# timothijoe/LightZero

Measured on AMD Instinct MI355X. Metric: MCTS simulations/sec (whole node), 256 parallel envs x 50 sims/step, higher is better.
Workload: dtype f32; 1 GPU; CartPole-v0 MuZero search, MuZeroModelMLP (latent 128, support 601), 256 envs x 50 sims per GPU; global_batch=256, num_simulations=50, rng=glibc, step=graph, hip_graph=True, heads=random, parallelism=env-sharded x1

## Files before the change

lightzero_amd/csrc/lzm_search_res.h:

```cpp
#pragma once
#include <hip/hip_runtime.h>
#include <stdint.h>

#include "lzm_search_mlp.h"
#include "lzm_tree.h"

namespace lzm {

constexpr int kRT = 256;
constexpr int kRWaves = kRT / 64;
constexpr int kRHid = 128, kRF = 32, kRV = 601;
constexpr int kRMaxA = 32;
constexpr int kRTail = kRV - 2 * kRT;
static_assert(kRTail > 0 && 2 * kRTail <= kRT, "support tail: two lanes per column");
constexpr int kRSlotsD = 16, kRSlotsRH = 4, kRSlotsVPH = 8, kRSlotsS = 20, kRSlotsPO = 1;

constexpr int kDwinBack = 20;

__device__ __forceinline__ void dwin_add_part(const uint32_t *coef, int npos, const uint32_t *z0, int lo, uint32_t *win,
                                              int part) {
  const int lane = threadIdx.x & 63;
  const int q = lo + lane;
  const int j0 = 11 * part, j1 = part == 2 ? 31 : j0 + 11;
  if (q < npos) {
// ... 628 lines not shown
    const int d = (lane == 0 && tv > 0) ? tv : tv + 1;
    const float y = div_small_y(d), nd = -(float)d;
    const bool below = lane < pend;
    float qv = parent_q;
    for (int i = pend; i < upto; ++i) {
      const float in = __int_as_float(__builtin_amdgcn_update_dpp(0, __float_as_int(qv), 0x138, 0xF, 0xF, true));
      const float q = div_small_core(in + tq, y, nd);
      qv = below ? qv : q;
    }
    const unsigned long long range = (~0ull >> (64 - (upto - pend))) << pend;
    const unsigned long long bad = __builtin_amdgcn_ballot_w64(__builtin_amdgcn_classf(tq, 0x020) ||
                                                               __builtin_amdgcn_classf(qv, sgpr_literal<0x207>()));
    if ((bad & range) == 0ull) return readlane_f(qv, upto - 1);
    parent_q = pend > 0 ? readlane_f(qv, pend - 1) : 0.0f;
  }
  const auto level = [&](int l, float &tq) {
    const int Ls = __builtin_amdgcn_readlane(plev, l);
    tq = readlane_f(rtq, Ls);
    return (__builtin_amdgcn_readlane(rpk, Ls) >> 5) & 3;
  };
  int l = pend;
  if (l == 0) {
    float tq;
    const int tv = level(0, tq);
    parent_q = div_small(tv > 0 ? tq : parent_q + tq, tv > 0 ? tv : 1);
    l = 1;
  }
  for (; l < upto; ++l) {
    float tq;
    const int tv = level(l, tq);
    parent_q = div_small(parent_q + tq, tv + 1);
  }
  return parent_q;
}

template <bool CLASSIFY, typename Draw>
__device__ inline Descent descend_a2r(const TreeView &t, const A2Rec &rc, bool leaf_ok, float4 mm, int vtp, int players,
                                      const int *rleg, int nleg, Draw draw, TieInfo *tie, WalkState *at_tie = nullptr) {
  const int lane = threadIdx.x & 63;
  const int dmax = t.depth_cap - 1;
  const int lat0 = __builtin_amdgcn_readfirstlane(t.meta[0].latent);
  int lat = lat0, len = 0;
  int plev = 0, pact = 0;
  float parent_q = 0.0f;
  int pend = 0;
  const auto rl = [](int v, int l) { return __builtin_amdgcn_readlane(v, l); };
  const auto rlf = [](float v, int l) { return __int_as_float(__builtin_amdgcn_readlane(__float_as_int(v), l)); };
  const auto child = [](int pk, int j) { return (int)((unsigned)pk << (8 - 8 * j)) >> 24; };
  const auto decided = [](int pk) { return (int)((unsigned)pk << 16) >> 24; };
  auto step = [&](int action, int nlat) {
    plev = lane == len ? lat : plev;
    pact = lane == len ? action : pact;
    ++len;
    lat = nlat;
  };
  const auto plat_of = [&]() { return len > 0 ? rl(plev, len - 1) : -1; };
  const auto act_of = [&]() { return len > 0 ? rl(pact, len - 1) : -1; };
  auto settle = [&](int upto) {
    parent_q = settle_chain(rc.tq, rc.pk, plev, leaf_ok, pend, upto, parent_q);
    pend = upto > pend ? upto : pend;
  };
  auto flush = [&]() {
    if (lane == 0) t.path[0] = 0;
    if (lane < len) {
      t.path_act[lane] = pact;
      t.path[lane + 1] = 1 + 2 * plev + pact;
    }
  };
  if (CLASSIFY) tie->status = 0;
  int pk = 0, dl = 0;
  bool stop = false;
  if (lat >= 0 && len < dmax) {
    pk = rl(rc.pk, lat);
    dl = pk & 7;
    if (dl <= 1)
      step(rleg[dl], decided(pk));
    else
      stop = true;
  }
  for (;;) {
    if (!stop && lat >= 0) {
      for (;;) {
        pk = rl(rc.pk, lat);
        dl = pk & 7;
        if (dl > 1) {
          stop = true;
          break;
        }
        step(dl, decided(pk));
        if (lat < 0) break;
      }
    }
    if (!stop || len >= dmax) break;
    stop = false;
    const bool root = len == 0;
    int jsel = 0;
    if (dl == 4 && leaf_ok) {
      if (CLASSIFY) {
        flush();
        const int vt = (players > 1 && (len & 1)) ? ((vtp == 1) ? 2 : 1) : vtp;
        tie->status = 1;
        tie->level = len;
        tie->mask = 3ull;
        Descent d;
        d.len = len + 1;
        d.x = lat;
        d.action = -1;
        d.vtp = players > 1 ? ((vt == 1) ? 2 : 1) : vt;
        d.leaf = -1;
        return d;
      }
      jsel = __builtin_amdgcn_readfirstlane((int)(draw(len) % 2u));
    } else {
      settle(len);
      bool tie2 = dl == 3;
      float mean_q = 0.0f;
      if (dl != 3) {
        const float delta = mm.x - mm.y;
        const bool scale = delta > 0;
        const float div = (delta < mm.z) ? mm.z : delta;
        const float tq = rlf(rc.tq, lat);
        const int tv = (pk >> 5) & 3;
        const bool rootq = root && tv > 0;
        mean_q = div_small(rootq ? tq : parent_q + tq, rootq ? tv : tv + 1);
        float vu = mm_norm_fixed(scale, mm.y, div, mean_q);
        if (vu < 0) vu = 0;
        if (vu > 1) vu = 1;
        const float s0 = rlf(rc.x0, lat) + ((pk & 8) ? rlf(rc.y0, lat) : vu);
        const float s1 = rlf(rc.x1, lat) + ((pk & 16) ? rlf(rc.y1, lat) : vu);
        const float M = fmaxf(s0, s1);
        const int j = (s0 == M) ? 0 : 1;
        jsel = __builtin_amdgcn_readfirstlane(j);
        tie2 = __builtin_amdgcn_readfirstlane((j == 0 && s1 >= M - 0.000001f) ? 1 : 0) != 0;
      }
      if (CLASSIFY && tie2) {
        const int vt = (players > 1 && (len & 1)) ? ((vtp == 1) ? 2 : 1) : vtp;
        const bool all_leaves = ((unsigned)pk >> 16) == 0xffffu;
        if (at_tie && !all_leaves) {
          const int plat = plat_of(), last_action = act_of();
          at_tie->node = root ? 0 : 1 + 2 * plat + last_action; at_tie->lat = lat; at_tie->len = len; at_tie->plat = plat;
          at_tie->last_action = last_action; at_tie->is_root = root; at_tie->vtp = vt; at_tie->parent_q = parent_q;
        }
        flush();
        tie->status = all_leaves ? 1 : 2;
        tie->level = len;
        tie->mask = 3ull;
        Descent d;
        d.len = len + 1;
        d.x = lat;
        d.action = -1;
        d.vtp = players > 1 ? ((vt == 1) ? 2 : 1) : vt;
        d.leaf = -1;
        return d;
      }
      if (!CLASSIFY && tie2) jsel = __builtin_amdgcn_readfirstlane((int)(draw(len) % 2u));
      if (dl != 3) {
        parent_q = mean_q;
        pend = len + 1;
      }
    }
    step(root ? rleg[jsel] : jsel, child(pk, jsel));
  }
  flush();
  const int plat = plat_of(), last_action = act_of();
  Descent d;
  d.len = len;
  d.x = plat;
  d.action = last_action;
  d.vtp = (players > 1 && (len & 1)) ? ((vtp == 1) ? 2 : 1) : vtp;
  d.leaf = len == 0 ? 0 : 1 + 2 * plat + last_action;
  return d;
}

struct NoSide {
  __device__ __forceinline__ void operator()(int) const {}
};
template <int NR, typename WF, typename SF = NoSide>
__device__ __forceinline__ void dense128n(const float *x, WF w, float *z, SF side = SF()) {
  const int e = threadIdx.x & 7;
  float4 xv[NR][4];
#pragma unroll
  for (int r = 0; r < NR; ++r)
#pragma unroll
    for (int j = 0; j < 4; ++j) xv[r][j] = reinterpret_cast<const float4 *>(x + r * kRRow)[4 * e + (e >> 2) + j];
  float a[NR][4][4];
#pragma unroll
  for (int r = 0; r < NR; ++r)
#pragma unroll
    for (int c = 0; c < 4; ++c) a[r][c][0] = a[r][c][1] = a[r][c][2] = a[r][c][3] = 0.0f;
#pragma unroll
  for (int j = 0; j < 4; ++j)
#pragma unroll
    for (int c = 0; c < 4; ++c) {
      side(4 * j + c);
      const float4 q = w(4 * j + c);
#pragma unroll
      for (int r = 0; r < NR; ++r) fma4(xv[r][j], q, a[r][c]);
    }
#pragma unroll
  for (int r = 0; r < NR; ++r)
    z[r] = reduce_d4((a[r][0][0] + a[r][0][1]) + (a[r][0][2] + a[r][0][3]),
                     (a[r][1][0] + a[r][1][1]) + (a[r][1][2] + a[r][1][3]),
                     (a[r][2][0] + a[r][2][1]) + (a[r][2][2] + a[r][2][3]),
                     (a[r][3][0] + a[r][3][1]) + (a[r][3][2] + a[r][3][3]));
}

template <int NH>
__device__ __forceinline__ void support_decode_n(const float (*z)[3], float *red, float *out) {
  const int tid = threadIdx.x, lane = tid & 63, wid = tid >> 6;
  const bool ok2 = tid < 2 * kRTail && !(tid & 1);
#pragma unroll
  for (int h = 0; h < NH; ++h) {
    float m = fmaxf(z[h][0], z[h][1]);
    if (ok2) m = fmaxf(m, z[h][2]);
    m = wave_max_dpp(m);
    if (lane == 0) red[4 * h + wid] = m;
  }
  __syncthreads();
  const float half = (float)((kRV - 1) / 2);
  const float j0 = (float)tid - half, j1 = (float)(kRT + tid) - half, j2 = (float)(2 * kRT + (tid >> 1)) - half;
#pragma unroll
  for (int h = 0; h < NH; ++h) {
    const float M = fmaxf(fmaxf(red[4 * h], red[4 * h + 1]), fmaxf(red[4 * h + 2], red[4 * h + 3]));
    const float e0 = expf(z[h][0] - M), e1 = expf(z[h][1] - M), e2 = ok2 ? expf(z[h][2] - M) : 0.0f;
    float se = (e0 + e1) + e2, sj = (e0 * j0 + e1 * j1) + e2 * j2;
    se = wave_sum(se);
    sj = wave_sum(sj);
    if (lane == 0) {
      red[4 * NH + 8 * h + wid] = se;
      red[4 * NH + 8 * h + 4 + wid] = sj;
    }
  }
  __syncthreads();
#pragma unroll
  for (int h = 0; h < NH; ++h) {
    const float *q = red + 4 * NH + 8 * h;
    out[h] = h_inverse(((q[4] + q[5]) + (q[6] + q[7])) / ((q[0] + q[1]) + (q[2] + q[3])));
  }
}

__device__ inline void resolve_tie(const TreeView &t, int A, int lvl, unsigned long long m, uint32_t rr, int *act) {
  int kk = (int)(rr % (uint32_t)__popcll(m));
  for (; kk > 0; --kk) m &= m - 1;
  const int jsel = __ffsll((long long)m) - 1;
  const int parent = t.path[lvl];
  const int action = legal_at(t, 0, parent, jsel);
  t.path_act[lvl] = action;
  t.path[lvl + 1] = 1 + A * t.meta[parent].latent + action;
  *act = action;
}

__device__ inline int lookback_sum(const SearchArgs &p, int k, int g, int G, unsigned long long epoch, int *part) {
  const int lane = threadIdx.x & 63;
  int sum = 0;
  for (int q = threadIdx.x; q < g; q += kRT) {
    unsigned long long v;
    long long spins = 0;
    while (true) {
      v = __hip_atomic_load(&p.flags[(size_t)k * G + q], __ATOMIC_RELAXED, __HIP_MEMORY_SCOPE_AGENT);
      if ((v >> 32) == epoch) break;
      if (++spins > (1ll << 22)) {
        atomicAdd(p.diag, 1);
        v = 0;
        break;
      }
      __builtin_amdgcn_s_sleep(1);
    }
    sum += (int)(v & 0xffffffffu);
  }
  sum = xor_sum(sum);
  if (lane == 0) part[threadIdx.x >> 6] = sum;
  __syncthreads();
  return (part[0] + part[1]) + (part[2] + part[3]);
}

__device__ inline int lookback_sum_w0(const SearchArgs &p, int k, int g, int G, unsigned long long epoch) {
  const int lane = threadIdx.x & 63;
  const unsigned long long ok = epoch << 32;
  unsigned long long v[4];
#pragma unroll
  for (int j = 0; j < 4; ++j) {
    const int q = lane + 64 * j;
    v[j] = q < g ? __hip_atomic_load(&p.flags[(size_t)k * G + q], __ATOMIC_RELAXED, __HIP_MEMORY_SCOPE_AGENT) : ok;
  }
  float sum = 0.0f;
#pragma unroll
  for (int j = 0; j < 4; ++j) {
    const int q = lane + 64 * j;
    long long spins = 0;
    while ((v[j] >> 32) != epoch) {
      if (++spins > (1ll << 22)) {
        atomicAdd(p.diag, 1);
        v[j] = ok;
        break;
      }
      __builtin_amdgcn_s_sleep(1);
      v[j] = __hip_atomic_load(&p.flags[(size_t)k * G + q], __ATOMIC_RELAXED, __HIP_MEMORY_SCOPE_AGENT);
    }
    sum += (float)(int)(v[j] & 0xffffffffu);
  }
  return (int)wave_sum(sum);
}

constexpr int kResStaticBytes = (kRRow + 4 * kRRow + 2 * (4 * kRRow + kRF + 2 * kRF + kRMaxA) + kResBiasFloats) * 4 + 2048;
constexpr int kResMaxBytes = 160 * 1024 - kResStaticBytes;
__host__ __device__ constexpr int res_round4(int x) { return (x + 3) & ~3; }
__host__ __device__ constexpr ResPlan res_plan(int cap, int lut_n, int depth_cap, int S, int A) {
  ResPlan q{};
  int o = 0;
  q.wd1 = o; o += kRSlotsD * kRT * 4;
  q.wd2 = o; o += kRSlotsD * kRT * 4;
  q.stat = o; o += cap * 4;
  q.meta = o; o += cap * 4;
  q.lut = o; o += res_round4(2 * lut_n);
  q.legal = o; o += res_round4(A + 1);
  q.val = o; o += res_round4(cap);
  q.path = o; o += res_round4(depth_cap);
  q.pact = o; o += res_round4(depth_cap);
  q.act = o; o += A * kRHid;
  q.l2n = o; o += res_round4(S + 2);
  q.nq = o; o += res_round4(2 * (S + 2));
  q.cs = o; o += 4 * cap;
  q.dec = o; o += res_round4(S + 2);
  q.misc = o; o += res_round4(S + 32);
  const int tri = res_round4(lut_n * (lut_n + 1) / 2);
  q.pbt = o;
  q.pbt_rows = ((o + tri) * 4 <= kResMaxBytes && tri <= 8192) ? lut_n : 0;
  if (q.pbt_rows) o += tri;
  q.floats = o;
  return q;
}

template <int SMODE, int RNG, bool STAMPS>
__global__ __launch_bounds__(kRT) __attribute__((amdgpu_waves_per_eu(1, 1))) void search_res_kernel(SearchArgs p, ResNet n) {
  if (!STAMPS) p.phase = nullptr;
  if (RNG >= 0) p.fast = RNG;
  const ResPlan L = n.plan;
  static_assert(SMODE == 1 || SMODE == 4 || SMODE == 5, "selection modes: 1, 4, 5");
  if ((SMODE == 4 || SMODE == 5) && RNG == 0 && !STAMPS) n.spec_depth = 1;
  extern __shared__ float4 smem4[];
  float *smem = reinterpret_cast<float *>(smem4);
  const int tid = threadIdx.x, g = blockIdx.x, G = gridDim.x, lane = tid & 63, wid = tid >> 6;
  const int B = p.B, A = p.A;
  const int i = g;
  unsigned long long stamp_ = p.phase ? __builtin_amdgcn_s_memtime() : 0ull;
  unsigned long long isub_ = stamp_;
#define LZM_ISTAMP(n)                                                      \
  do {                                                                     \
    if (p.phase && tid == 0) {                                             \
      const unsigned long long now_ = __builtin_amdgcn_s_memtime();       \
      s_phase[n] += (now_ - isub_) * (unsigned long long)p.S;              \
      isub_ = now_;                                                        \
    }                                                                      \
  } while (0)

  __shared__ uint32_t s_z0[31];
  __shared__ int s_players, s_epoch, s_x, s_act, s_status, s_tlevel, s_vtp;
  __shared__ int s_len[1], s_part[kRWaves], s_nlat;
  __shared__ unsigned long long s_tmask;
  __shared__ WalkState s_walk;
  __shared__ float4 s_mm;
  __shared__ float s_red[12 * 2];
  __shared__ uint32_t s_dwin[64];
  __shared__ int s_dlo, s_base_prev;
  if (tid == 0) { s_dlo = -1000000; s_base_prev = 0; }
  __shared__ uint64_t s_exptab[32];
  if (threadIdx.x < 32) s_exptab[threadIdx.x] = kExp2fTab[threadIdx.x];
  __shared__ unsigned long long s_phase[64];
  if (p.phase && tid < 64) s_phase[tid] = 0ull;
  unsigned long long s_wait = 0ull;

  TreeView t;
  t.A = A; t.cap = p.cap; t.lut_n = p.lut_n; t.depth_cap = p.depth_cap; t.B = 1;
  t.path = reinterpret_cast<int32_t *>(smem + L.path);
  t.path_act = reinterpret_cast<int32_t *>(smem + L.pact);
  t.pathlen = s_len;
  {
    NodeStat *ls = reinterpret_cast<NodeStat *>(smem + L.stat);
    NodeMeta *lm = reinterpret_cast<NodeMeta *>(smem + L.meta);
    float2 *llut = reinterpret_cast<float2 *>(smem + L.lut);
    int32_t *llegal = reinterpret_cast<int32_t *>(smem + L.legal);
    float *lval = smem + L.val;
    for (int e = tid; e < p.cap; e += kRT) {
      const NodeStat s = p.stat[(size_t)e * B + i];
      ls[e] = s;
      lm[e] = p.meta[(size_t)e * B + i];
      lval[e] = node_value(s);
    }
    for (int e = tid; e < p.lut_n; e += kRT) llut[e] = p.lut[e];
    float *lpbt = smem + L.pbt;
    build_pbt(p.lut, p.pbt_rows, lpbt, tid, kRT);
    for (int e = tid; e < A; e += kRT) llegal[e] = p.legal[(size_t)i * A + e];
    if (tid == 0) llegal[A] = p.nlegal[i];
    t.stat = ls; t.meta = lm; t.lut = llut; t.legal = llegal; t.nlegal = llegal + A; t.val = lval;
    t.pbt = p.pbt_rows ? lpbt : nullptr;
  }
  LZM_ISTAMP(24);
  int *L2N = reinterpret_cast<int *>(smem + L.l2n);
  float2 *NQ = reinterpret_cast<float2 *>(smem + L.nq);
  int *DEC = reinterpret_cast<int *>(smem + L.dec);
  float4 *CS = reinterpret_cast<float4 *>(smem + L.cs);
  for (int e = tid; e < p.S + 2; e += kRT) L2N[e] = e == 0 ? 0 : -1;
  if (tid == 0) s_nlat = 1;
  if (tid == 0) {
    s_mm = p.mm_fresh ? make_float4(kFloatMin, kFloatMax, p.mm_delta, 0.0f) : p.minmax[i];
    s_vtp = p.vtp_in[i];
    s_epoch = (int)__hip_atomic_load(p.epoch, __ATOMIC_RELAXED, __HIP_MEMORY_SCOPE_AGENT);
  }
  if (wid == 0) {
    int m = INT_MIN;
    for (int q = lane; q < B; q += 64) m = max(m, p.vtp_in[q]);
    m = xor_max(m);
    if (lane == 0) s_players = (m == -1) ? 1 : 2;
  }
  uint32_t *s_seeds = reinterpret_cast<uint32_t *>(smem + L.misc);
  uint32_t *s_pow = s_seeds + p.S;
  if (p.step_count) {
    const long long c = *p.step_count;
    for (int e = tid; e < p.S; e += kRT) s_seeds[e] = (uint32_t)((p.step_base + c * (long long)p.S + e) % 1000000ll);
  } else {
    for (int e = tid; e < p.S; e += kRT) s_seeds[e] = p.seeds[e];
  }
  if (!p.fast)
    for (int e = tid; e < 31; e += kRT) s_pow[e] = p.pow16807[e];

  LZM_ISTAMP(25);
  __shared__ float4 s_acts[(kRRow + 4 * kRRow + 4 * kRRow + kRF + 2 * kRF + kRMaxA) / 4];
  __shared__ float4 s_bias[kResBiasFloats / 4];
  float *X0 = reinterpret_cast<float *>(s_acts), *T1 = X0 + kRRow, *NL = T1 + 2 * kRRow, *T2 = NL + 2 * kRRow,
        *T3 = T2 + kRRow, *U2 = T3 + kRRow, *U3 = U2 + kRRow, *RHo = U3 + kRRow, *HV = RHo + kRF, *LG = HV + 2 * kRF;
  float *ACT = smem + L.act;
  const float4 *WD1 = reinterpret_cast<const float4 *>(smem + L.wd1);
  const float4 *WD2 = reinterpret_cast<const float4 *>(smem + L.wd2);
  {
    float4 st[kRSlotsD];
    res_fetch<kRSlotsD>(res_blk4(n, kRbD + 1), st);
#pragma unroll
    for (int j = 0; j < kRSlotsD; ++j) reinterpret_cast<float4 *>(smem + L.wd1)[j * kRT + tid] = st[j];
    res_fetch<kRSlotsD>(res_blk4(n, kRbD + 2), st);
#pragma unroll
    for (int j = 0; j < kRSlotsD; ++j) reinterpret_cast<float4 *>(smem + L.wd2)[j * kRT + tid] = st[j];
  }
  for (int e = tid; e < A * kRHid; e += kRT) ACT[e] = res_blk(n, kRbAct, A)[e];
  LZM_ISTAMP(26);
  float4 wD3[kRSlotsD], wD4[kRSlotsD], wRS[kRSlotsS], wRH[kRSlotsRH], wVPH[kRSlotsVPH], wPO[1];
  res_fetch<kRSlotsD>(res_blk4(n, kRbD + 3), wD3);
  res_fetch<kRSlotsD>(res_blk4(n, kRbD + 4), wD4);
  res_fetch<kRSlotsS>(res_blk4(n, kRbRS), wRS);
  res_fetch<kRSlotsRH>(res_blk4(n, kRbRH), wRH);
  res_fetch<kRSlotsVPH>(res_blk4(n, kRbVPH), wVPH);
  res_fetch<kRSlotsPO>(res_blk4(n, kRbPO), wPO);
  const int cD = d_col(), pD = tid & 1, cRH = tid >> 3, pRH = tid & 7, cVP = tid >> 2, pVP = tid & 3, cPO = tid >> 3;
  LZM_ISTAMP(27);
  float *BB = reinterpret_cast<float *>(s_bias);
  {
    constexpr int kNB = (kResBiasFloats + kRT - 1) / kRT;
    float bv[kNB];
    const float *bsrc = res_blk(n, kRbBD, A);
#pragma unroll
    for (int j = 0; j < kNB; ++j) bv[j] = j * kRT + tid < kResBiasFloats ? bsrc[j * kRT + tid] : 0.0f;
#pragma unroll
    for (int j = 0; j < kNB; ++j)
      if (j * kRT + tid < kResBiasFloats) BB[j * kRT + tid] = bv[j];
  }
  const float *BD = BB, *BRH = BD + 6 * kRHid, *BVP = BRH + kRF, *BRS = BVP + 2 * kRF,
              *BVS = BRS + ((kRV + 3) & ~3), *BPO = BVS + ((kRV + 3) & ~3);
  float4 P[kRSlotsS];
  res_fetch<kRSlotsD>(res_blk4(n, kRbD), P);
#pragma unroll
  for (int j = kRSlotsD; j < kRSlotsS; ++j) P[j] = make_float4(0.0f, 0.0f, 0.0f, 0.0f);
  __syncthreads();
  const int players = s_players;
  const unsigned long long epoch = (unsigned long long)(uint32_t)s_epoch;
  int rleg[2];
  const int nleg = t.nlegal[0];
#pragma unroll
  for (int j = 0; j < 2; ++j) rleg[j] = j < A ? t.legal[j] : 0;
  LZM_ISTAMP(28);
  LZM_STAMP(10);

  for (int k = 0; k < p.S; ++k) {
    const uint32_t seed = s_seeds[k];
    const bool regwalk = SMODE == 5;
    const int smode = regwalk ? 4 : (SMODE == 4 && A != 2) ? 1 : SMODE;
    A2Rec rc = {0, 0.0f, 0.0f, 0.0f, 0.0f, 0.0f};
    __syncthreads();
    if (regwalk) {
      if (tid < s_nlat + k) node_terms_a2(t, tid, L2N, NQ, CS, s_mm, players, p.disc, DEC, rleg, nleg, &rc);
    } else {
      if (smode == 4)
        precompute_terms_a2(t, s_nlat + k, L2N, NQ, CS, s_mm, players, p.disc, DEC, rleg, nleg);
      else
        precompute_terms(t, s_nlat + k, L2N, NQ, CS, s_mm, players, p.disc);
      __syncthreads();
    }
    LZM_STAMP(12);
    if (wid != 0 && k > 0) res_fetch<kRSlotsD>(res_blk4(n, kRbD), P);
    if (!p.fast && wid == 1) {
      const uint32_t sd = seed == 0 ? 1u : seed;
      if (sd < 0x7fffffffu) {
        if (lane < 31) {
          unsigned long long x = (unsigned long long)sd * s_pow[lane];
          unsigned long long r = (x & 0x7fffffffull) + (x >> 31);
          r = (r & 0x7fffffffull) + (r >> 31);
          if (r >= 0x7fffffffull) r -= 0x7fffffffull;
          s_z0[lane] = (uint32_t)r;
        }
      } else if (lane == 0) {
        glibc_seed_state(seed, s_z0);
      }
    }
    if (RNG != 1 && wid == 1) s_dwin[lane] = 0u;
    if (wid == 0) {
      const float4 mm = s_mm;
      int w_status = 0, w_x = 0;
      if (p.fast) {
        auto draw = [seed, i](int level) -> uint32_t {
          uint4 o = philox4x32_10(make_uint4((uint32_t)level, (uint32_t)i, 0u, 0u), make_uint2(seed, 0x4c5a4d43u));
          return o.x >> 1;
        };
        Descent d;
        if (regwalk) {
          d = descend_a2r<false>(t, rc, terms_finite_a2r(rc, mm), mm, s_vtp, players, rleg, nleg, draw, nullptr);
          w_x = d.x;
        } else if (smode == 4) {
          d = descend_a2f<false>(t, NQ, DEC, CS, mm, s_vtp, players, rleg, nleg, draw, nullptr);
        } else if (smode == 1) {
          d = descend_terms<false>(t, NQ, CS, mm, s_vtp, players, draw, nullptr);
        }
        if (lane == 0) { s_len[0] = d.len; s_x = d.x; s_act = d.action; s_status = 0; }
      } else {
        TieInfo ti;
        auto nodraw = [](int) -> uint32_t { return 0u; };
        Descent d;
        if (regwalk) {
          WalkState ws;
          d = descend_a2r<true>(t, rc, terms_finite_a2r(rc, mm), mm, s_vtp, players, rleg, nleg, nodraw, &ti, &ws);
          LZM_STAMP(13);
          if (lane == 0 && ti.status == 2) s_walk = ws;
          w_status = ti.status;
          w_x = d.x;
        } else if (smode == 4) {
          WalkState ws;
          d = descend_a2f<true>(t, NQ, DEC, CS, mm, s_vtp, players, rleg, nleg, nodraw, &ti, &ws);
          LZM_STAMP(13);
          if (lane == 0 && ti.status == 2) s_walk = ws;
        } else if (smode == 1) {
          WalkState ws;
          d = descend_terms<true>(t, NQ, CS, mm, s_vtp, players, nodraw, &ti, nullptr, &ws);
          if (lane == 0 && ti.status == 2) s_walk = ws;
        }
        if (lane == 0) {
          s_len[0] = d.len; s_x = d.x; s_act = d.action;
          s_status = ti.status; s_tlevel = ti.level; s_tmask = ti.mask;
          if (ti.status != 2)
            __hip_atomic_store(&p.flags[(size_t)k * G + g], (epoch << 32) | (unsigned)d.len, __ATOMIC_RELAXED,
                               __HIP_MEMORY_SCOPE_AGENT);
        }
      }
      if (!regwalk) {
        __builtin_amdgcn_fence(__ATOMIC_RELEASE, "wavefront");
        __builtin_amdgcn_wave_barrier();
        __builtin_amdgcn_fence(__ATOMIC_ACQUIRE, "wavefront");
      }
      const int stw = __builtin_amdgcn_readfirstlane(regwalk ? w_status : s_status);
      const int x0 = __builtin_amdgcn_readfirstlane(regwalk ? w_x : s_x);
      if (stw != 2 && lane < kRHid / 4)
        reinterpret_cast<float4 *>(X0)[lane + (lane >= kRHid / 8)] =
            reinterpret_cast<const float4 *>(p.pool + ((size_t)max(x0, 0) * B + i) * kRHid)[lane];
    }
    __syncthreads();
    LZM_STAMP(0);
    const int status = s_status;
    if (__builtin_expect(status == 2, 0)) {
      int st = 2, d0 = -1;
      uint32_t sp_choice = ~0u, sp_ties = 0u;
      int sp_leaf = -1;
      unsigned long long sub_ = p.phase ? __builtin_amdgcn_s_memtime() : 0ull;
      if (smode == 4 && n.spec_depth && wid == 0) {
        const int de = speculate_depth_a2(t, NQ, DEC, CS, s_mm, rleg, nleg, s_walk, lane, &sp_choice, &sp_ties, &sp_leaf);
        d0 = __builtin_amdgcn_readfirstlane(de);
        if (d0 >= 0 && __ballot(de != d0) == 0ull) {
          st = 3;
          if (lane == 0)
            __hip_atomic_store(&p.flags[(size_t)k * G + g], (epoch << 32) | (unsigned)d0, __ATOMIC_RELAXED,
                               __HIP_MEMORY_SCOPE_AGENT);
        }
      }
      LZM_SUBSTAMP(20);
      const bool win2 = RNG != 1 && smode == 4 && G <= kRT;
      int base = 0;
      if (win2) {
        if (wid == 0) {
          base = lookback_sum_w0(p, k, g, G, epoch);
        } else {
          const int lo = max(s_base_prev - kDwinBack, 0);
          dwin_add_part(p.coef, p.coef_positions, s_z0, lo, s_dwin, wid - 1);
          if (tid == 64) s_dlo = lo;
        }
        __syncthreads();
      } else {
        base = lookback_sum(p, k, g, G, epoch, s_part);
      }
      LZM_SUBSTAMP(21);
      if (wid == 0) {
        if (lane == 0) atomicAdd(p.diag + (st == 2 ? 1 : 2), 1);
        WalkState ws = s_walk;
        const int hi = st == 3 ? d0 : t.depth_cap;
        bool need = true;
        uint32_t wv = 0u;
        if (win2) {
          bool miss;
          wv = window_draw(p.coef_positions, base, ws.len, hi, s_dwin, s_dlo, &miss);
          need = __ballot(miss) != 0ull;
          if (lane == 0) s_base_prev = base;
          if (p.phase && lane == 0 && need) s_phase[41] += 1;
        }
        if (need) {
          const int q = base + ws.len + lane;
          wv = 0u;
          if (ws.len + lane < hi && q < p.coef_positions) {
            const uint32_t *c = p.coef + (size_t)q * 31;
#pragma unroll
            for (int j = 0; j < 31; ++j) wv += c[j] * s_z0[j];
            wv >>= 1;
          }
        }
        const LaneDraws draw{p.coef, s_z0, p.diag, p.coef_positions, base, ws.len, wv};
        Descent d;
        int m = -1;
        uint32_t pch = 0u;
        if (st == 3 && smode == 4) {
          const unsigned long long par = __ballot((wv & 1u) != 0u);
          const bool ok = sp_choice != ~0u && ((sp_choice ^ (uint32_t)par) & sp_ties) == 0u;
          const unsigned long long okm = __ballot(ok);
          if (okm) {
            m = __ffsll((long long)okm) - 1;
            pch = (uint32_t)__builtin_amdgcn_readlane((int)sp_choice, m);
            const int lt = __builtin_amdgcn_readlane(sp_leaf, m);
            if (lt >= 0) pch = (pch & ~(1u << lt)) | ((uint32_t)(par >> lt) & 1u) << lt;
          }
        }
        if (m >= 0) {
          int node = ws.node, lat = ws.lat, len = ws.len, plat = ws.plat, last_action = ws.last_action;
          const int dmax = t.depth_cap - 1;
          while (lat >= 0 && len < dmax) {
            const bool root = node == 0;
            const int j = (int)((pch >> (len - ws.len)) & 1u);
            const int action = j ? (root ? rleg[1] : 1) : (root ? rleg[0] : 0);
            const int nnode = 1 + 2 * lat + action;
            const int nlat = __float_as_int(CS[nnode].z);
            if (lane == 0) {
              t.path_act[len] = action;
              t.path[len + 1] = nnode;
            }
            ++len;
            plat = lat;
            lat = nlat;
            node = nnode;
            last_action = action;
          }
          d.len = len;
          d.x = plat;
          d.action = last_action;
          d.vtp = 0;
          d.leaf = node;
        } else if (smode == 4)
          d = descend_a2<false>(t, NQ, DEC, CS, s_mm, s_vtp, players, rleg, nleg, draw, nullptr, &ws);
        else
          d = descend_terms<false>(t, NQ, CS, s_mm, s_vtp, players, draw, nullptr, &ws);
        if (lane == 0) {
          if (st == 3 && d.len != d0) {
            atomicAdd(p.diag, 1);
            atomicAdd(p.diag + 3, 1);
          }
          s_len[0] = d.len; s_x = d.x; s_act = d.action;
          if (st == 2)
            __hip_atomic_store(&p.flags[(size_t)k * G + g], (epoch << 32) | (unsigned)d.len, __ATOMIC_RELAXED,
                               __HIP_MEMORY_SCOPE_AGENT);
        }
        const int x0 = __builtin_amdgcn_readfirstlane(d.x);
        if (lane < kRHid / 4)
          reinterpret_cast<float4 *>(X0)[lane + (lane >= kRHid / 8)] =
              reinterpret_cast<const float4 *>(p.pool + ((size_t)max(x0, 0) * B + i) * kRHid)[lane];
      }
      LZM_SUBSTAMP(22);
      __syncthreads();
      LZM_SUBSTAMP(23);
    }
    LZM_STAMP(1);
    LZM_STAMP(2);
    unsigned long long sub_ = p.phase ? __builtin_amdgcn_s_memtime() : 0ull;
    const float z0 = dense128(X0, [&](int j) { return P[j]; });
    __builtin_amdgcn_sched_barrier(0);
#pragma unroll
    for (int j = 0; j < kRSlotsD; ++j) P[j] = WD1[j * kRT + tid];
    LZM_SUBSTAMP(16);
    bool late = false;
    int act_r[2];
    if (status == 1) {
      const unsigned long long m = s_tmask;
      const int parent = t.path[s_tlevel];
      if (__popcll(m) == 2 && n.late_draw) {
        late = true;
        act_r[0] = legal_at(t, 0, parent, __ffsll((long long)m) - 1);
        act_r[1] = legal_at(t, 0, parent, __ffsll((long long)(m & (m - 1))) - 1);
      } else {
        const int base = lookback_sum(p, k, g, G, epoch, s_part);
        if (tid == 0) resolve_tie(t, A, s_tlevel, m, glibc_draw(p.coef, p.coef_positions, s_z0, base + s_tlevel, p.diag), &s_act);
        __syncthreads();
      }
    }
    if (!late) act_r[0] = act_r[1] = s_act;
    LZM_SUBSTAMP(17);
    __builtin_amdgcn_sched_barrier(0);
    if (pD == 0) {
#pragma unroll
      for (int r = 0; r < 2; ++r)
        if (r < 1 || late) T1[r * kRRow + rpad(cD)] = fmaxf((z0 + ACT[act_r[r] * kRHid + cD]) + BD[cD], 0.0f);
    }
    __syncthreads();
    LZM_SUBSTAMP(18);
    if (late) {
      float z[2];
      dense128n<2>(T1, [&](int j) { return P[j]; }, z);
      LZM_SUBSTAMP(32);
      if (pD == 0) {
#pragma unroll
        for (int r = 0; r < 2; ++r) NL[r * kRRow + rpad(cD)] = fmaxf(z[r] + BD[kRHid + cD], 0.0f) + X0[rpad(cD)];
      }
    } else {
      float z;
      dense128n<1>(T1, [&](int j) { return P[j]; }, &z);
      if (pD == 0) NL[rpad(cD)] = fmaxf(z + BD[kRHid + cD], 0.0f) + X0[rpad(cD)];
    }
    __syncthreads();
    LZM_SUBSTAMP(33);
    int lrow = 0;
    if (late) {
      const unsigned long long w0_ = p.phase ? __builtin_amdgcn_s_memtime() : 0ull;
      if (G <= kRT) {
        const int base = lookback_sum_w0(p, k, g, G, epoch);
        if (p.phase && tid == 0) s_wait += __builtin_amdgcn_s_memtime() - w0_;
        const uint32_t rr = glibc_draw_wave(p.coef, p.coef_positions, s_z0, base + s_tlevel, p.diag);
        lrow = (int)(rr & 1u);
        if (tid == 0) resolve_tie(t, A, s_tlevel, s_tmask, rr, &s_act);
      } else {
        const int base = lookback_sum(p, k, g, G, epoch, s_part);
        if (p.phase && tid == 0) s_wait += __builtin_amdgcn_s_memtime() - w0_;
        if (tid == 0) resolve_tie(t, A, s_tlevel, s_tmask, glibc_draw(p.coef, p.coef_positions, s_z0, base + s_tlevel, p.diag), &s_act);
        __syncthreads();
        lrow = s_act == act_r[1] ? 1 : 0;
      }
    }
    const float *NLb = NL + ((late && lrow) ? kRRow : 0);
    LZM_SUBSTAMP(34);
    LZM_STAMP(3);
    {
      float z2, z6;
      const __amdgpu_buffer_rsrc_t rd5 = wave_rsrc(res_blk4(n, kRbD + 5), kRSlotsD * kRT * 16);
      dense128n<1>(NLb, [&](int j) { return WD2[j * kRT + tid]; }, &z2, [&](int j) {
        const f32x4 v = __builtin_amdgcn_raw_buffer_load_b128(rd5, tid * 16, j * kRT * 16, 0);
        P[j] = make_float4(v.x, v.y, v.z, v.w);
      });
      LZM_SUBSTAMP(35);
      dense128n<1>(NLb, [&](int j) { return wD4[j]; }, &z6);
      LZM_SUBSTAMP(36);
      if (pD == 0) {
        T2[rpad(cD)] = fmaxf(z2 + BD[2 * kRHid + cD], 0.0f);
        U2[rpad(cD)] = fmaxf(z6 + BD[4 * kRHid + cD], 0.0f);
      }
    }
    __syncthreads();
    LZM_SUBSTAMP(19);
    {
      float z7, z3;
      dense128n<1>(U2, [&](int j) { return P[j]; }, &z7);
      LZM_SUBSTAMP(37);
      __builtin_amdgcn_sched_barrier(0);
      const __amdgpu_buffer_rsrc_t rvs = wave_rsrc(res_blk4(n, kRbVS), kRSlotsS * kRT * 16);
      auto fetch_vs = [&](int q0, int q1) {
#pragma unroll
        for (int q = q0; q < q1; ++q) {
          const f32x4 v = __builtin_amdgcn_raw_buffer_load_b128(rvs, tid * 16, q * kRT * 16, 0);
          P[q] = make_float4(v.x, v.y, v.z, v.w);
        }
      };
      fetch_vs(0, kRSlotsS / 2);
      dense128n<1>(T2, [&](int j) { return wD3[j]; }, &z3);
      LZM_SUBSTAMP(38);
      __builtin_amdgcn_sched_barrier(0);
      fetch_vs(kRSlotsS / 2, kRSlotsS);
      if (pD == 0) {
        T3[rpad(cD)] = fmaxf(z3 + BD[3 * kRHid + cD], 0.0f);
        U3[rpad(cD)] = fmaxf(z7 + BD[5 * kRHid + cD], 0.0f);
      }
    }
    __syncthreads();
    LZM_SUBSTAMP(39);
    LZM_STAMP(4);
    {
      float h = dot4<kRSlotsRH>(reinterpret_cast<const float4 *>(T3) + 4 * pRH + (pRH >= 4), [&](int j) { return wRH[j]; });
      float u = dot4<kRSlotsVPH>(reinterpret_cast<const float4 *>(U3) + 8 * pVP + (pVP >= 2), [&](int j) { return wVPH[j]; });
      h += dpp_f<0xB1>(h);
      u += dpp_f<0xB1>(u);
      h += dpp_f<0x4E>(h);
      u += dpp_f<0x4E>(u);
      h += dpp_f<0x141>(h);
      if (pRH == 0) RHo[cRH] = fmaxf(h + BRH[cRH], 0.0f);
      if (pVP == 0) HV[cVP] = fmaxf(u + BVP[cVP], 0.0f);
    }
    __syncthreads();
    LZM_STAMP(5);
    float dec[2];
    {
      float zz[2][3];
      const float4 hp = reinterpret_cast<const float4 *>(HV + kRF)[tid & 7];
      float q = __fmaf_rn(hp.x, wPO[0].x, 0.0f);
      q = __fmaf_rn(hp.y, wPO[0].y, q);
      q = __fmaf_rn(hp.z, wPO[0].z, q);
      q = __fmaf_rn(hp.w, wPO[0].w, q);
      q += dpp_f<0xB1>(q);
      q += dpp_f<0x4E>(q);
      q += dpp_f<0x141>(q);
      if ((tid & 7) == 0 && cPO < A) LG[cPO] = q + BPO[cPO];
      support_logits(HV, P, BVS, zz[1][0], zz[1][1], zz[1][2]);
      __builtin_amdgcn_sched_barrier(0);
      support_logits(RHo, wRS, BRS, zz[0][0], zz[0][1], zz[0][2]);
      __builtin_amdgcn_sched_barrier(0);
      LZM_STAMP(15);
      support_decode_n<2>(zz, s_red, dec);
    }
    const float rdec = dec[0], vdec = dec[1];
    LZM_STAMP(6);
    LZM_STAMP(7);
    if (p.phase && tid == 0) sub_ = __builtin_amdgcn_s_memtime();
    if (tid >= 64 && tid < 64 + kRHid / 4)
      reinterpret_cast<float4 *>(p.pool + ((size_t)(k + 1) * B + i) * kRHid)[tid - 64] =
          reinterpret_cast<const float4 *>(NLb)[(tid - 64) + (tid - 64 >= kRHid / 8)];
    if (p.rec_x && tid == 0) {
      p.rec_x[(size_t)k * B + i] = s_x;
      p.rec_a[(size_t)k * B + i] = s_act;
      p.rec_len[(size_t)k * B + i] = s_len[0];
    }
    if (p.rec_dec && tid == 0) {
      p.rec_dec[((size_t)k * B + i) * 2] = rdec;
      p.rec_dec[((size_t)k * B + i) * 2 + 1] = vdec;
      for (int a = 0; a < A; ++a) p.rec_logits[((size_t)k * B + i) * A + a] = LG[a];
    }
    LZM_SUBSTAMP(29);
    if (wid == 0) res_fetch<kRSlotsD>(res_blk4(n, kRbD), P);
    LZM_SUBSTAMP(30);
    if (wid == 0) {
      const int len = s_len[0];
      const int leaf = t.path[len];
      int vtp = s_vtp;
      if (players > 1)
        for (int l = 0; l < len; ++l) vtp = (vtp == 1) ? 2 : 1;
      LZM_SUBSTAMP(31);
      expand_wave(t, 0, leaf, vtp, k + 1, rdec, LG, -1, s_exptab, 1);
      LZM_STAMP(14);
      if (lane == 0) L2N[s_nlat + k] = leaf;
      backup_wave(t, 0, 0, 1, &s_mm, vtp, vdec, p.disc);
    } else if (wid == 1) {
      expand_wave(t, 0, 0, 0, k + 1, 0.0f, LG, -1, s_exptab, 2);
    }
    LZM_STAMP(9);
  }
  __syncthreads();
  LZM_STAMP(11);
  for (int e = tid; e < p.cap; e += kRT) {
    p.stat[(size_t)e * B + i] = t.stat[e];
    p.meta[(size_t)e * B + i] = t.meta[e];
  }
  for (int e = tid; e < p.depth_cap; e += kRT) {
    p.path[(size_t)e * B + i] = t.path[e];
    p.path_act[(size_t)e * B + i] = t.path_act[e];
  }
  if (tid == 0) {
    p.minmax[i] = s_mm;
    p.pathlen[i] = s_len[0];
  }
  if (p.out_dist && tid < A) {
    const int rl = t.meta[0].latent;
    p.out_dist[(size_t)i * A + tid] = (rl >= 0 && tid < t.nlegal[0]) ? t.stat[1 + A * rl + t.legal[tid]].visit : -1;
  }
  if (p.out_values && tid == 0) p.out_values[i] = node_value(t.stat[0]);
  __syncthreads();
  if (p.phase && tid < 64 && s_phase[tid]) atomicAdd(p.phase + tid, s_phase[tid]);
  if (p.phase && tid == 0 && g < 1024) atomicAdd(p.phase + 64 + g, s_wait);
  if (tid == 0) {
    const uint32_t done = atomicAdd(p.epoch + 1, 1u);
    if (done == (uint32_t)G - 1) {
      p.epoch[1] = 0;
      __hip_atomic_store(p.epoch, (uint32_t)(epoch + 1), __ATOMIC_RELAXED, __HIP_MEMORY_SCOPE_AGENT);
      if (p.step_count && p.step_inc) *p.step_count += 1;
    }
  }
}

}
```

Before: 26.93 million sims/s.

## Pack descent handoff into one shared word and specialize regwalk expand/backup

On the register-walk path, the descent result (status, length, leaf index, action) is packed into a single shared int that is broadcast with readfirstlane, in place of several separate shared variables. Tie resolution for the two-action case is computed directly from the packed data, writing the path entry arithmetically. It also adds specialized expand and backup routines that load the path once per lane and do the backup with readlane scans, skipping the generic tree walk. The packing assumes length, leaf index and action each fit in 8 bits, and the vtp parity and leaf formula assume a fixed binary tree layout, which adds correctness risk.

Result: faster. 27.56 million sims/s, median of 6 (+2.3%).

```diff
diff --git a/lightzero_amd/csrc/lzm_search_res.h b/lightzero_amd/csrc/lzm_search_res.h
--- a/lightzero_amd/csrc/lzm_search_res.h
+++ b/lightzero_amd/csrc/lzm_search_res.h
@@ -954,6 +954,82 @@
   return (int)wave_sum(sum);
 }
 
+__device__ __forceinline__ int hand_pack(int status, int len, int x, int action) {
+  return (status & 3) | ((len & 0xff) << 2) | ((x & 0xff) << 10) | ((action & 0xff) << 18);
+}
+struct HandOff {
+  int status, len, x, action;
+};
+__device__ __forceinline__ HandOff hand_unpack(int w) {
+  HandOff h;
+  h.status = w & 3;
+  h.len = (w >> 2) & 0xff;
+  h.x = (int)((unsigned)w << 14) >> 24;
+  h.action = (int)((unsigned)w << 6) >> 24;
+  return h;
+}
+
+struct TailPath {
+  int node, pact;
+};
+__device__ inline TailPath expand_wave_r(const TreeView &t, int len, int leaf, int to_play, int latent, float reward) {
+  const int lane = threadIdx.x & 63;
+  const int lv = min(lane, t.depth_cap - 1);
+  TailPath tp;
+  tp.node = t.path[lv];
+  tp.pact = t.path_act[lv];
+  tp.node = lane <= len ? tp.node : 0;
+  if (lane == 0) {
+    t.meta[leaf].latent = latent;
+    t.meta[leaf].to_play = to_play;
+    t.stat[leaf].reward = reward;
+  }
+  return tp;
+}
+__device__ inline void backup_wave_r(const TreeView &t, const TailPath &tp, int len, int to_play, float value,
+                                     float disc, float4 *mm_ptr) {
+  const int lane = threadIdx.x & 63;
+  const int node = tp.node;
+  const bool act = lane <= len;
+  if (lane < len) t.meta[node].best = tp.pact;
+  NodeStat s = t.stat[node];
+  const int ntp = t.meta[node].to_play;
+  float b = value;
+  float bl = 0.0f;
+  for (int j = len; j >= 0; --j) {
+    if (lane == j) bl = b;
+    const float tr = readlane_f(s.reward, j);
+    if (to_play == -1) {
+      b = tr + disc * b;
+    } else {
+      const int nj = __builtin_amdgcn_readlane(ntp, j);
+      b = (nj == to_play) ? (-tr + disc * b) : (tr + disc * b);
+    }
+  }
+  float qmax = -INFINITY, qmin = INFINITY;
+  if (act) {
+    if (to_play == -1 || ntp == to_play)
+      s.value_sum += bl;
+    else
+      s.value_sum += -bl;
+    s.visit += 1;
+    t.stat[node] = s;
+    const float v = node_value(s);
+    if (t.val) t.val[node] = v;
+    const float q = (to_play == -1) ? s.reward + disc * v : s.reward + disc * -v;
+    qmax = fmaxf(qmax, q);
+    qmin = fminf(qmin, q);
+  }
+  qmax = wave_max_dpp(qmax);
+  qmin = -wave_max_dpp(-qmin);
+  if (lane == 0) {
+    float4 mm = *mm_ptr;
+    if (qmax > mm.x) mm.x = qmax;
+    if (qmin < mm.y) mm.y = qmin;
+    *mm_ptr = mm;
+  }
+}
+
 constexpr int kResStaticBytes = (kRRow + 4 * kRRow + 2 * (4 * kRRow + kRF + 2 * kRF + kRMaxA) + kResBiasFloats) * 4 + 2048;
 constexpr int kResMaxBytes = 160 * 1024 - kResStaticBytes;
 __host__ __device__ constexpr int res_round4(int x) { return (x + 3) & ~3; }
@@ -1009,6 +1085,7 @@
   __shared__ uint32_t s_z0[31];
   __shared__ int s_players, s_epoch, s_x, s_act, s_status, s_tlevel, s_vtp;
   __shared__ int s_len[1], s_part[kRWaves], s_nlat;
+  __shared__ int s_hand;
   __shared__ unsigned long long s_tmask;
   __shared__ WalkState s_walk;
   __shared__ float4 s_mm;
@@ -1180,7 +1257,13 @@
         } else if (smode == 1) {
           d = descend_terms<false>(t, NQ, CS, mm, s_vtp, players, draw, nullptr);
         }
-        if (lane == 0) { s_len[0] = d.len; s_x = d.x; s_act = d.action; s_status = 0; }
+        if (lane == 0) {
+          if (regwalk) {
+            s_hand = hand_pack(0, d.len, d.x, d.action);
+          } else {
+            s_len[0] = d.len; s_x = d.x; s_act = d.action; s_status = 0;
+          }
+        }
       } else {
         TieInfo ti;
         auto nodraw = [](int) -> uint32_t { return 0u; };
@@ -1203,8 +1286,11 @@
           if (lane == 0 && ti.status == 2) s_walk = ws;
         }
         if (lane == 0) {
-          s_len[0] = d.len; s_x = d.x; s_act = d.action;
-          s_status = ti.status; s_tlevel = ti.level; s_tmask = ti.mask;
+          if (regwalk) s_hand = hand_pack(ti.status, d.len, d.x, d.action);
+          if (!regwalk || ti.status == 2) {
+            s_len[0] = d.len; s_x = d.x; s_act = d.action;
+            s_status = ti.status; s_tlevel = ti.level; s_tmask = ti.mask;
+          }
           if (ti.status != 2)
             __hip_atomic_store(&p.flags[(size_t)k * G + g], (epoch << 32) | (unsigned)d.len, __ATOMIC_RELAXED,
                                __HIP_MEMORY_SCOPE_AGENT);
@@ -1223,7 +1309,9 @@
     }
     __syncthreads();
     LZM_STAMP(0);
-    const int status = s_status;
+    HandOff ho = {0, 0, 0, 0};
+    if (regwalk) ho = hand_unpack(__builtin_amdgcn_readfirstlane(s_hand));
+    const int status = regwalk ? ho.status : s_status;
     if (__builtin_expect(status == 2, 0)) {
       int st = 2, d0 = -1;
       uint32_t sp_choice = ~0u, sp_ties = 0u;
@@ -1327,6 +1415,7 @@
             atomicAdd(p.diag + 3, 1);
           }
           s_len[0] = d.len; s_x = d.x; s_act = d.action;
+          if (regwalk) s_hand = hand_pack(2, d.len, d.x, d.action);
           if (st == 2)
             __hip_atomic_store(&p.flags[(size_t)k * G + g], (epoch << 32) | (unsigned)d.len, __ATOMIC_RELAXED,
                                __HIP_MEMORY_SCOPE_AGENT);
@@ -1338,6 +1427,7 @@
       }
       LZM_SUBSTAMP(22);
       __syncthreads();
+      if (regwalk) ho = hand_unpack(__builtin_amdgcn_readfirstlane(s_hand));
       LZM_SUBSTAMP(23);
     }
     LZM_STAMP(1);
@@ -1350,7 +1440,26 @@
     LZM_SUBSTAMP(16);
     bool late = false;
     int act_r[2];
-    if (status == 1) {
+    const int tlevel = regwalk ? ho.len - 1 : 0;
+    if (regwalk) {
+      if (status == 1) {
+        act_r[0] = tlevel == 0 ? rleg[0] : 0;
+        act_r[1] = tlevel == 0 ? rleg[1] : 1;
+        if (n.late_draw) {
+          late = true;
+        } else {
+          const int base = lookback_sum(p, k, g, G, epoch, s_part);
+          const uint32_t rr = glibc_draw_wave(p.coef, p.coef_positions, s_z0, base + tlevel, p.diag);
+          ho.action = (rr & 1u) ? act_r[1] : act_r[0];
+          if (tid == 0) {
+            t.path_act[tlevel] = ho.action;
+            t.path[tlevel + 1] = 1 + 2 * ho.x + ho.action;
+            s_act = ho.action;
+          }
+        }
+      }
+      if (!late) act_r[0] = act_r[1] = ho.action;
+    } else if (status == 1) {
       const unsigned long long m = s_tmask;
       const int parent = t.path[s_tlevel];
       if (__popcll(m) == 2 && n.late_draw) {
@@ -1363,7 +1472,7 @@
         __syncthreads();
       }
     }
-    if (!late) act_r[0] = act_r[1] = s_act;
+    if (!regwalk && !late) act_r[0] = act_r[1] = s_act;
     LZM_SUBSTAMP(17);
     __builtin_amdgcn_sched_barrier(0);
     if (pD == 0) {
@@ -1391,7 +1500,25 @@
     int lrow = 0;
     if (late) {
       const unsigned long long w0_ = p.phase ? __builtin_amdgcn_s_memtime() : 0ull;
-      if (G <= kRT) {
+      if (regwalk) {
+        uint32_t rr;
+        if (G <= kRT) {
+          const int base = lookback_sum_w0(p, k, g, G, epoch);
+          if (p.phase && tid == 0) s_wait += __builtin_amdgcn_s_memtime() - w0_;
+          rr = glibc_draw_wave(p.coef, p.coef_positions, s_z0, base + tlevel, p.diag);
+        } else {
+          const int base = lookback_sum(p, k, g, G, epoch, s_part);
+          if (p.phase && tid == 0) s_wait += __builtin_amdgcn_s_memtime() - w0_;
+          rr = glibc_draw_wave(p.coef, p.coef_positions, s_z0, base + tlevel, p.diag);
+        }
+        lrow = (int)(rr & 1u);
+        ho.action = lrow ? act_r[1] : act_r[0];
+        if (tid == 0) {
+          t.path_act[tlevel] = ho.action;
+          t.path[tlevel + 1] = 1 + 2 * ho.x + ho.action;
+          s_act = ho.action;
+        }
+      } else if (G <= kRT) {
         const int base = lookback_sum_w0(p, k, g, G, epoch);
         if (p.phase && tid == 0) s_wait += __builtin_amdgcn_s_memtime() - w0_;
         const uint32_t rr = glibc_draw_wave(p.coef, p.coef_positions, s_z0, base + s_tlevel, p.diag);
@@ -1491,9 +1618,9 @@
       reinterpret_cast<float4 *>(p.pool + ((size_t)(k + 1) * B + i) * kRHid)[tid - 64] =
           reinterpret_cast<const float4 *>(NLb)[(tid - 64) + (tid - 64 >= kRHid / 8)];
     if (p.rec_x && tid == 0) {
-      p.rec_x[(size_t)k * B + i] = s_x;
-      p.rec_a[(size_t)k * B + i] = s_act;
-      p.rec_len[(size_t)k * B + i] = s_len[0];
+      p.rec_x[(size_t)k * B + i] = regwalk ? ho.x : s_x;
+      p.rec_a[(size_t)k * B + i] = regwalk ? ho.action : s_act;
+      p.rec_len[(size_t)k * B + i] = regwalk ? ho.len : s_len[0];
     }
     if (p.rec_dec && tid == 0) {
       p.rec_dec[((size_t)k * B + i) * 2] = rdec;
@@ -1503,7 +1630,21 @@
     LZM_SUBSTAMP(29);
     if (wid == 0) res_fetch<kRSlotsD>(res_blk4(n, kRbD), P);
     LZM_SUBSTAMP(30);
-    if (wid == 0) {
+    if (regwalk && wid == 0) {
+      const int len = ho.len;
+      const int leaf = len > 0 ? 1 + 2 * ho.x + ho.action : 0;
+      int vtp = s_vtp;
+      if (players > 1 && len > 0) {
+        vtp = (vtp == 1) ? 2 : 1;
+        if ((len - 1) & 1) vtp = (vtp == 1) ? 2 : 1;
+      }
+      LZM_SUBSTAMP(31);
+      const TailPath tp = expand_wave_r(t, len, leaf, vtp, k + 1, rdec);
+      LZM_STAMP(14);
+      if (lane == 0) L2N[s_nlat + k] = leaf;
+      backup_wave_r(t, tp, len, vtp, vdec, p.disc, &s_mm);
+      if (lane == 0) { s_len[0] = len; s_x = ho.x; s_act = ho.action; }
+    } else if (wid == 0) {
       const int len = s_len[0];
       const int leaf = t.path[len];
       int vtp = s_vtp;
```
